# pengpeng-yu/FastPCC

Hardware: AMD Instinct MI355X
Metric: encode+decode Mpoints/sec, lossy_coord_v2 baseline_r1 (stream of 16-frame batches, 2 in flight; one frame at a time = value_one_frame) (higher is better)
Workload: dtype f32; 1 GPU; lossy_coord_v2/baseline_r1 inference, 997645-voxel 1024^3 body-surface frames (cfg#2), seeded random-init weights; one step = a batch of 16 such frames per GPU (15966320 voxels) through compress_many + decompress_many = ONE network traversal over the batch, 16 independent streams; 2 batch(es) in flight per GPU; parallelism=single GPU, 2 batches in flight per GPU on one stream (fastpcc_amd/serving.py), batch_clouds=16, frames_in_flight=2, named_stages=False, bytes=143901, coder_handover_retries=0

## Files before the change

fastpcc_amd/csrc/hip/conv.hip:

```cpp
#include "conv_common.h"
#include <atomic>
#include <cstdlib>

namespace fpcc {
namespace {

template <int NBT, int CH, int WM, int WN>
struct MfmaCfg {
    static constexpr int C_OUT = 32 * NBT;
    static constexpr int TM = 32 * WM;
    static constexpr int NBW = NBT / WN;
    static constexpr int THREADS = 64 * WM * WN;
    static constexpr int G8 = CH / 8;
    static constexpr int W_TOTAL = CH * C_OUT / 4;
    static constexpr int W_PIECES = (W_TOTAL + THREADS - 1) / THREADS;
    static_assert(NBT % WN == 0, "column blocks must divide over the waves");
};

template <typename C, int CH>
__device__ __forceinline__ void fetch_a(const ConvArgs &a, const int32_t *nbr_rows, int cc, int li, int lh,
                                        f32x4 (&ra)[C::G8]) {
    const bool in_x1 = cc * CH < a.c1;
    const float *xb = in_x1 ? a.x1 + cc * CH : a.x2 + (cc * CH - a.c1);
    const int64_t ld = in_x1 ? a.ld1 : a.ld2;
// ... 640 lines not shown
        }
        __builtin_amdgcn_sched_barrier(0);
        for (int s = 0; s < n_stages; ++s) {
            next_stage();
            __builtin_amdgcn_sched_barrier(SB);
#pragma unroll
            for (int g8 = 0; g8 < G8; ++g8) {
                const f32x4 av0 = ra[0][g8], av1 = ra[1][g8];
                const f32x4 b0 = rbv[g8][0], b1 = rbv[g8][1];
#define FPCC_STEP(c)                                                                                     \
                acc[0][0] = __builtin_amdgcn_mfma_f32_32x32x2f32(av0.c, b0.c, acc[0][0], 0, 0, 0);       \
                acc[0][1] = __builtin_amdgcn_mfma_f32_32x32x2f32(av0.c, b1.c, acc[0][1], 0, 0, 0);       \
                acc[1][0] = __builtin_amdgcn_mfma_f32_32x32x2f32(av1.c, b0.c, acc[1][0], 0, 0, 0);       \
                acc[1][1] = __builtin_amdgcn_mfma_f32_32x32x2f32(av1.c, b1.c, acc[1][1], 0, 0, 0);
                FPCC_STEP(x) FPCC_STEP(y) FPCC_STEP(z) FPCC_STEP(w)
#undef FPCC_STEP
                __builtin_amdgcn_sched_barrier(SB);
                ra[0][g8] = *reinterpret_cast<const f32x4 *>(ap[0] + 8 * g8);
                __builtin_amdgcn_sched_barrier(SB);
                ra[1][g8] = *reinterpret_cast<const f32x4 *>(ap[1] + 8 * g8);
#pragma unroll
                for (int nb = 0; nb < 2; ++nb) {
                    __builtin_amdgcn_sched_barrier(SB);
                    rbv[g8][nb] = *reinterpret_cast<const f32x4 *>(bp + ((int64_t)g8 * nbt + nb) * 256);
                }
                __builtin_amdgcn_sched_barrier(SB);
            }
        }
    }

    const float slope = (a.act == FPCC_ACT_PRELU && a.slope) ? a.slope[0] : 0.0f;
    float bias2[2];
#pragma unroll
    for (int nb = 0; nb < 2; ++nb) bias2[nb] = a.bias ? a.bias[32 * ((int)cg * 2 + nb) + li] : 0.0f;
#pragma unroll
    for (int rb = 0; rb < 2; ++rb) {
        int64_t dsts[16];
#pragma unroll
        for (int reg = 0; reg < 16; ++reg) {
            const int64_t o = __shfl(my_row, 32 * rb + (reg & 3) + 8 * (reg >> 2) + 4 * lh);
            dsts[reg] = o < 0 ? -1 : a.out_map ? (int64_t)a.out_map[o * a.om_os + g * a.om_gs] : o * a.groups + g;
        }
#pragma unroll
        for (int reg = 0; reg < 16; ++reg) {
            const int64_t dst = dsts[reg];
            if (dst < 0) continue;
#pragma unroll
            for (int nb = 0; nb < 2; ++nb)
                a.out[dst * a.ldo + 32 * ((int)cg * 2 + nb) + li] = finish(acc[rb][nb][reg], bias2[nb], a.act, slope, a.clip);
        }
    }
}

__global__ __launch_bounds__(256) void k_pack_weights(const float *__restrict__ w, int64_t n_mats, int c_in, int c_out,
                                                      float *__restrict__ wp) {
    const int64_t e = (int64_t)blockIdx.x * 256 + threadIdx.x;
    const int64_t per_mat = (int64_t)c_in * c_out;
    if (e >= n_mats * per_mat) return;
    const int nbt = c_out / 32;
    const int64_t m = e / per_mat;
    int64_t r = e - m * per_mat;
    const int j = (int)(r & 3); r >>= 2;
    const int i = (int)(r & 31); r >>= 5;
    const int h = (int)(r & 1); r >>= 1;
    const int nb = (int)(r % nbt); r /= nbt;
    const int g8 = (int)(r & 3); r >>= 2;
    const int cc = (int)r;
    wp[e] = w[m * per_mat + (int64_t)(32 * cc + 8 * g8 + 4 * h + j) * c_out + 32 * nb + i];
}

inline bool aligned16(const void *p) { return (reinterpret_cast<uintptr_t>(p) & 15) == 0; }

int mfma_chunk(int c1, int c2, int c_out) {
    if (c_out != 32 && c_out != 64 && c_out != 128) return 0;
    const int c_in = c1 + c2;
    if (c_in % 32 == 0 && c1 % 32 == 0) return 32;
    if (c_in % 16 == 0 && c1 % 16 == 0) return 16;
    return 0;
}

int knob(int k);

template <int NBT, int CH, int WM, int WN>
int launch_mfma_cfg(ConvArgs a, hipStream_t s) {
    constexpr int TM = 32 * WM;
    const unsigned tiles = (unsigned)((a.n_out + TM - 1) / TM);
    const dim3 grid(tiles, a.groups), block(64 * WM * WN);
    hipLaunchKernelGGL((k_conv_mfma<NBT, CH, WM, WN>), grid, block, 0, s, a);
    return check_hip(hipGetLastError(), "k_conv_mfma");
}

enum { kKnobWaveOn = 0, kKnobWaveNbw = 1, kKnobWaveSb = 2, kKnobStamps = 3, kKnobGroupedFoldRows = 4, kKnobMfmaCfg = 5, kKnobPointwiseRows = 6,
       kKnobGroupedOff = 7, kKnobGroupedNbw = 8, kKnobWave22Rows = 9, kKnobLdsRows = 10, kKnobLdsRowBlocks = 11, kKnobPersist = 12, kKnobCount = 13 };
int g_knob[kKnobCount] = {-1, -1, -1, -1, -1, -1, -1, -1, -1, -1, -1, -1, -1};
int knob(int k) {
    if (g_knob[k] < 0) {
        static const char *names[kKnobCount] = {"FPCC_CONV_WAVE", "FPCC_WAVE_NBW", "FPCC_WAVE_SB", "", "FPCC_GROUPED_FOLD_ROWS",
                                                "FPCC_MFMA_TILE", "FPCC_POINTWISE_MIN_ROWS", "", "FPCC_GROUPED_NBW",
                                                "FPCC_WAVE22_MIN_ROWS", "FPCC_LDS_MIN_ROWS", "FPCC_LDS_ROW_BLOCKS",
                                                "FPCC_CONV_PERSIST"};
        static const int defaults[kKnobCount] = {1, 0, 1, 0, 100 * 1024, 0, 32 * 1024, 0, 0, 0, 0, 2, 0};
        const char *e = names[k][0] ? getenv(names[k]) : nullptr;
        g_knob[k] = e ? atoi(e) : defaults[k];
    }
    return g_knob[k];
}

template <int NBT, int CH>
int launch_mfma(const ConvArgs &a, hipStream_t s) {
    const int forced = knob(kKnobMfmaCfg) - 1;
    const int64_t work = a.n_out * a.groups;
    constexpr int WNS = NBT >= 2 ? 2 : 1;
    const int cfg = forced >= 0 ? forced : (NBT <= 2 && work >= 128 * 1024) ? 0 : work >= 32 * 1024 ? 1 : 2;
    if (cfg == 0) return launch_mfma_cfg<NBT, CH, 4, 1>(a, s);
    if (cfg == 1) return launch_mfma_cfg<NBT, CH, 2, WNS>(a, s);
    return launch_mfma_cfg<NBT, CH, 1, NBT>(a, s);
}

__global__ __launch_bounds__(256) void k_conv_c1_pointwise(ConvArgs a) {
    const int64_t e = (int64_t)blockIdx.x * 256 + threadIdx.x;
    if (e >= a.n_out * a.c_out) return;
    const int64_t o = e / a.c_out;
    const int j = (int)(e - o * a.c_out);
    const float slope = (a.act == FPCC_ACT_PRELU && a.slope) ? a.slope[0] : 0.0f;
    a.out[o * a.ldo + j] = finish(fmaf(a.x1[o * a.ld1], a.w[j], 0.0f), a.bias ? a.bias[j] : 0.0f, a.act, slope, a.clip);
}

template <int NBW>
int launch_wave_cfg(const ConvArgs &a, const float *wp, int nbt, hipStream_t s) {
    const int64_t row_blocks = (a.n_out + 31) / 32;
    const int64_t units = row_blocks * (nbt / NBW);
    if (units > 0x7fffffffll) return fail_arg("conv_f32: too many work units");
    const dim3 grid((unsigned)((units + 3) / 4), a.groups);
    if (knob(kKnobWaveSb)) hipLaunchKernelGGL((k_conv_wave<NBW, 32, 0x6>), grid, dim3(256), 0, s, a, wp, nbt, (unsigned)units);
    else hipLaunchKernelGGL((k_conv_wave<NBW, 32, 0>), grid, dim3(256), 0, s, a, wp, nbt, (unsigned)units);
    return check_hip(hipGetLastError(), "k_conv_wave");
}

constexpr int kMaxDevices = 16;
inline int current_device() {
    int dev = 0;
    return (hipGetDevice(&dev) == hipSuccess && dev >= 0 && dev < kMaxDevices) ? dev : -1;
}
int cu_count() {
    static std::atomic<int> cached[kMaxDevices];
    const int dev = current_device();
    if (dev < 0) return 256;
    int n = cached[dev].load(std::memory_order_relaxed);
    if (n == 0) {
        hipDeviceProp_t prop;
        n = (hipGetDeviceProperties(&prop, dev) == hipSuccess && prop.multiProcessorCount > 0) ? prop.multiProcessorCount : 256;
        cached[dev].store(n, std::memory_order_relaxed);
    }
    return n;
// ... 21 lines not shown
    *rc = check_hip(hipMemsetD32Async(reinterpret_cast<hipDeviceptr_t>(c), (int)start, 1, s), "unit counter fill");
    return c;
}

inline int64_t persist_slots() {
    const int v = knob(kKnobPersist);
    return v > 16 ? v : (int64_t)v * cu_count();
}
inline bool persist_ok(const ConvArgs &a) {
    return knob(kKnobPersist) > 0 && a.nbr && a.nbr_ks == 1 && (a.nbr_os & 3) == 0 && a.nbr_os >= ((a.n_off + 3) & ~3) &&
           (reinterpret_cast<uintptr_t>(a.nbr) & 15) == 0 && a.groups == 1;
}

template <int NBW>
int launch_grouped_cfg(const ConvArgs &a, const float *wp, int nbt, hipStream_t s) {
    const int64_t row_blocks = (a.n_out + 31) / 32;
    const int64_t units = row_blocks * (nbt / NBW);
    if (units > 0x7fffffffll) return fail_arg("conv_f32: too many work units");
    const bool stamps = knob(kKnobStamps) != 0;
    const int64_t slots = persist_slots();
    if (!stamps && persist_ok(a) && units > slots) {
        int rc = FPCC_OK;
        unsigned *counter = next_unit_counter((unsigned)slots, s, &rc);
        if (rc != FPCC_OK) return rc;
        hipLaunchKernelGGL((k_conv_wave<NBW, 32, 0x6, false, 4, false, true>), dim3((unsigned)slots, 1), dim3(256), 0, s, a, wp, nbt, (unsigned)units,
                           counter);
        return check_hip(hipGetLastError(), "k_conv_wave(grouped, persistent)");
    }
    if (stamps)
        hipLaunchKernelGGL((k_conv_wave<NBW, 32, 0x6, true, 4>), dim3((unsigned)units, a.groups), dim3(256), 0, s, a, wp, nbt, (unsigned)units);
    else
        hipLaunchKernelGGL((k_conv_wave<NBW, 32, 0x6, false, 4>), dim3((unsigned)units, a.groups), dim3(256), 0, s, a, wp, nbt, (unsigned)units);
    return check_hip(hipGetLastError(), "k_conv_wave(grouped)");
}

template <int NBW>
int launch_folded_cfg(const ConvArgs &a, const float *wp, int nbt, hipStream_t s) {
    const int64_t units = ((a.n_out + 31) / 32) * (nbt / NBW);
    if (units > 0x7fffffffll) return fail_arg("conv_f32: too many work units");
    const int64_t slots = persist_slots();
    if (!knob(kKnobStamps) && persist_ok(a) && (units + 3) / 4 > slots) {
        int rc = FPCC_OK;
        unsigned *counter = next_unit_counter((unsigned)(4 * slots), s, &rc);
        if (rc != FPCC_OK) return rc;
        hipLaunchKernelGGL((k_conv_wave<NBW, 32, 0x6, false, 1, true, true>), dim3((unsigned)slots, 1), dim3(256), 0, s, a, wp, nbt, (unsigned)units,
                           counter);
        return check_hip(hipGetLastError(), "k_conv_wave(folded, persistent)");
    }
    hipLaunchKernelGGL((k_conv_wave<NBW, 32, 0x6, false, 1, true>), dim3((unsigned)((units + 3) / 4), a.groups), dim3(256), 0, s, a, wp, nbt,
                       (unsigned)units);
    return check_hip(hipGetLastError(), "k_conv_wave(folded)");
}

int launch_grouped(const ConvArgs &a, const float *wp, hipStream_t s) {
    const int nbt = a.c_out / 32;
    const int64_t lds_rows = knob(kKnobLdsRows);
    if (lds_rows > 0 && a.n_out >= lds_rows) {
        const int rc = launch_conv_lds(a, wp, knob(kKnobLdsRowBlocks), knob(kKnobStamps) != 0, s);
        if (rc != -1) return rc;
    }
    const int64_t fold_rows = knob(kKnobGroupedFoldRows);
    if (fold_rows > 0 && a.n_out >= fold_rows && knob(kKnobGroupedNbw) <= 0)
        return nbt % 2 == 0 ? launch_folded_cfg<2>(a, wp, nbt, s) : launch_folded_cfg<1>(a, wp, nbt, s);
    int nbw = knob(kKnobGroupedNbw);
    if (nbw <= 0) nbw = a.n_out >= 40 * 1024 ? 2 : 1;
    while (nbw > nbt || nbt % nbw) nbw >>= 1;
    return nbw == 2 ? launch_grouped_cfg<2>(a, wp, nbt, s) : launch_grouped_cfg<1>(a, wp, nbt, s);
}

int launch_wave22(const ConvArgs &a, const float *wp, int nbt, hipStream_t s) {
    const int64_t units = ((a.n_out + 63) / 64) * (nbt / 2);
    if (units > 0x7fffffffll) return fail_arg("conv_f32: too many work units");
    const dim3 grid((unsigned)((units + 3) / 4), a.groups);
    if (knob(kKnobWaveSb)) hipLaunchKernelGGL((k_conv_wave22<0x6>), grid, dim3(256), 0, s, a, wp, nbt, (unsigned)units);
    else hipLaunchKernelGGL((k_conv_wave22<0>), grid, dim3(256), 0, s, a, wp, nbt, (unsigned)units);
    return check_hip(hipGetLastError(), "k_conv_wave22");
}

int launch_wave(const ConvArgs &a, const float *wp, hipStream_t s) {
    const int nbt = a.c_out / 32;
    const int64_t work = a.n_out * a.groups;
    const int64_t rows22 = knob(kKnobWave22Rows);
    if (rows22 > 0 && a.n_off > 1 && nbt % 2 == 0 && work >= rows22 && knob(kKnobWaveNbw) <= 0) return launch_wave22(a, wp, nbt, s);
    int nbw = knob(kKnobWaveNbw);
    if (nbw <= 0) nbw = work >= 32 * 1024 ? 2 : 1;
    while (nbw > nbt || nbt % nbw) nbw >>= 1;
    if (nbw >= 4) return launch_wave_cfg<4>(a, wp, nbt, s);
    if (nbw == 2) return launch_wave_cfg<2>(a, wp, nbt, s);
    return launch_wave_cfg<1>(a, wp, nbt, s);
}


template <int NBW, int NCH>
__global__ __launch_bounds__(256, 2) void k_pointwise_wave(ConvArgs a, const float *__restrict__ wp, int nbt, unsigned n_row_blocks,
                                                           unsigned waves_per_cg) {
    constexpr int AC = NCH < 4 ? NCH : 4;
    constexpr int TW = 32 * NBW + 4;
    __shared__ float s_tile[4][32 * TW];
    const int lane = threadIdx.x & 63, wv = threadIdx.x >> 6;
    const int li = lane & 31, lh = lane >> 5;
    const unsigned n_cg = (unsigned)(nbt / NBW);
    const unsigned w = blockIdx.x * 4u + (unsigned)wv;
    const unsigned cg = w % n_cg, slot = w / n_cg;
    if (slot >= waves_per_cg) return;

    f32x4 rb[NCH][4][NBW];
    {
        const float *wpl = wp + ((int64_t)cg * NBW) * 256 + lane * 4;
#pragma unroll
        for (int cc = 0; cc < NCH; ++cc)
#pragma unroll
            for (int g8 = 0; g8 < 4; ++g8)
#pragma unroll
                for (int nb = 0; nb < NBW; ++nb)
                    rb[cc][g8][nb] = *reinterpret_cast<const f32x4 *>(wpl + (((int64_t)cc * 4 + g8) * nbt + nb) * 256);
    }
// ... 183 lines not shown
    return check_hip(hipGetLastError(), "k_conv_valu");
}

}
}

using namespace fpcc;

static bool use_grouped(int c1, int c2, int c_out, int n_offsets, int groups) {
    return mfma_chunk(c1, c2, c_out) == 32 && n_offsets >= 8 && n_offsets <= kMaxOffsets && groups == 1 && !knob(kKnobGroupedOff);
}

extern "C" int fpcc_conv_f32_order(int c1, int c2, int c_out) { return mfma_chunk(c1, c2, c_out) ? 1 : 0; }

extern "C" int64_t fpcc_conv_f32_ws_bytes(int c1, int c2, int c_out, int n_offsets, int groups, int64_t n_out) {
    if (n_out > 0 && use_grouped(c1, c2, c_out, n_offsets, groups)) return (int64_t)n_offsets * (c1 + c2) * c_out * 4;
    return 0;
}

extern "C" int fpcc_conv_f32_order_ex(int c1, int c2, int c_out, int n_offsets, int groups, int64_t n_out) {
    (void)n_out;
    if (use_grouped(c1, c2, c_out, n_offsets, groups)) return 3;
    return mfma_chunk(c1, c2, c_out) ? 1 : 0;
}

extern "C" int fpcc_numerics_version(void) { return FPCC_NUMERICS_VERSION; }

extern "C" int fpcc_conv_ones_k3_f32(const uint32_t *masks, int64_t n, const float *w, const float *bias, int c_out, int act,
                                     const float *slope, float clip, float *out, int ldo, void *stream) {
    if (n < 0 || c_out < 4 || c_out > 32 || c_out % 4 || ldo < c_out || ldo % 4) return fail_arg("conv_ones_k3: 4 <= c_out <= 32, multiple of 4");
    if (n == 0) return FPCC_OK;
    if (!masks || !w || !out || !aligned16(out)) return fail_arg("conv_ones_k3: null or unaligned pointer");
    if (act == FPCC_ACT_PRELU && !slope) return fail_arg("conv_ones_k3: PReLU needs a slope pointer");
    hipStream_t st = as_stream(stream);
    switch (c_out) {
        case 4: return launch_ones_k3<4>(masks, n, w, bias, act, slope, clip, out, ldo, st);
        case 8: return launch_ones_k3<8>(masks, n, w, bias, act, slope, clip, out, ldo, st);
        case 12: return launch_ones_k3<12>(masks, n, w, bias, act, slope, clip, out, ldo, st);
        case 16: return launch_ones_k3<16>(masks, n, w, bias, act, slope, clip, out, ldo, st);
        case 20: return launch_ones_k3<20>(masks, n, w, bias, act, slope, clip, out, ldo, st);
        case 24: return launch_ones_k3<24>(masks, n, w, bias, act, slope, clip, out, ldo, st);
        case 28: return launch_ones_k3<28>(masks, n, w, bias, act, slope, clip, out, ldo, st);
        default: return launch_ones_k3<32>(masks, n, w, bias, act, slope, clip, out, ldo, st);
    }
}

extern "C" int fpcc_conv_debug_stamps(unsigned long long *buf, int64_t n_u64) {
    if (n_u64 < 0 || (n_u64 > 0 && !buf)) return fail_arg("conv_debug_stamps: null buffer");
    const long long cap = buf ? n_u64 : 0;
    FPCC_HIP(hipMemcpyToSymbol(HIP_SYMBOL(g_stamp_buf), &buf, sizeof(buf)));
    FPCC_HIP(hipMemcpyToSymbol(HIP_SYMBOL(g_stamp_cap), &cap, sizeof(cap)));
    return set_lds_stamp_buffer(buf, cap);
}

extern "C" int fpcc_conv_set_tuning(int which, int value) {
    if (which < 0 || which >= kKnobCount) return fail_arg("conv_set_tuning: unknown knob");
    if (which == kKnobGroupedOff) {
        const char *e = getenv("FPCC_EXPERIMENT");
        if (!e || atoi(e) != 1)
            return fail_arg("conv_set_tuning: the summation order is part of the stream format (FPCC_EXPERIMENT=1 to override)");
    }
    if (which == kKnobStamps && value != 0 && value != 16)
        return fail_arg("conv_set_tuning: knob 3 is 0 or 16 (stamped builds); the timing ablations are no longer part of the library");
    const int before = knob(which);
    g_knob[which] = value < 0 ? 0 : value;
    return before;
}

extern "C" int64_t fpcc_conv_packed_floats(int c1, int c2, int c_out, int n_offsets, int groups) {
    if (mfma_chunk(c1, c2, c_out) != 32 || n_offsets < 1 || n_offsets > kMaxOffsets || groups < 1) return 0;
    return (int64_t)groups * n_offsets * (c1 + c2) * c_out;
}

extern "C" int fpcc_conv_pack_weights_f32(const float *w, int64_t n_mats, int c_in, int c_out, float *w_packed, void *stream) {
    if (n_mats < 0 || c_in < 32 || c_in % 32 || (c_out != 32 && c_out != 64 && c_out != 128))
        return fail_arg("conv_pack_weights: c_in must be a multiple of 32 and c_out one of 32, 64, 128");
    if (n_mats == 0) return FPCC_OK;
    if (!w || !w_packed) return fail_arg("conv_pack_weights: null pointer");
    hipLaunchKernelGGL(k_pack_weights, dim3(blocks_for(n_mats * c_in * c_out, 256)), dim3(256), 0, as_stream(stream), w, n_mats,
                       c_in, c_out, w_packed);
    return check_hip(hipGetLastError(), "k_pack_weights");
}

extern "C" int fpcc_conv_f32(const float *x1, int c1, int ld1, const float *x2, int c2, int ld2, const int32_t *nbr,
                             int n_offsets, int64_t nbr_ks, int64_t nbr_os, const float *w, const float *bias, int c_out,
                             int groups, const int32_t *out_map, int64_t om_os, int64_t om_gs, float *out, int ldo,
                             int64_t n_out, int act, const float *slope, float clip, const int32_t *row_order,
                             void *ws, int64_t ws_bytes, void *stream) {
    return fpcc_conv_f32_pk(x1, c1, ld1, x2, c2, ld2, nbr, n_offsets, nbr_ks, nbr_os, w, nullptr, bias, c_out, groups, out_map,
                            om_os, om_gs, out, ldo, n_out, act, slope, clip, row_order, ws, ws_bytes, stream);
}

namespace fpcc {
PendingEvents &pending_events() {
    static thread_local PendingEvents p;
    return p;
}
}

extern "C" int fpcc_time_next_launch(void *start_event, void *end_event) {
    PendingEvents &p = pending_events();
    p.ev0 = start_event;
    p.ev1 = end_event;
    return FPCC_OK;
}

// ... 383 lines not shown
```

fastpcc_amd/hipops.py:

```python
import collections
import ctypes as C
import functools
from typing import List, Optional, Sequence, Tuple

import torch

from . import _native

_vp, _i64, _i32, _f32 = C.c_void_p, C.c_int64, C.c_int, C.c_float

ACT_NONE, ACT_PRELU, ACT_RELU = 0, 1, 2

_SIGS = {
    'fpcc_morton3d_encode': (_i32, [_vp, _i64, _i64, _i32, _i32, _i32, _vp, _vp]),
    'fpcc_hilbert3d_encode': (_i32, [_vp, _i64, _i64, _i32, _i32, _i32, _i32, _vp, _vp]),
    'fpcc_keys_from_coords': (_i32, [_vp, _i64, _i32, _i32, _vp, _vp]),
    'fpcc_coords_from_keys': (_i32, [_vp, _i64, _i32, _i32, _vp, _vp, _vp]),
    'fpcc_sort_keys': (_i64, [_vp, _i64, _i32, _vp, _vp, _vp, _i64, _vp]),
    'fpcc_unique_keys': (_i64, [_vp, _i64, _vp, _vp, _vp, _vp, _i64, _vp]),
    'fpcc_coarsen': (_i64, [_vp, _i64, _vp, _vp, _vp, _vp, _vp, _i64, _vp]),
    'fpcc_octree_level': (_i64, [_vp, _i64, _i64, _i32, _vp, _vp, _vp, _vp, _i64, _vp, _vp, _i64, _vp]),
    'fpcc_level_histogram': (_i64, [_vp, _i64, _i32, _vp, _vp]),
    'fpcc_level_histogram_clouds': (_i64, [_vp, _i64, _i32, _i32, _i32, _vp, _vp]),
    'fpcc_refine': (_i64, [_vp, _i64, _vp, _vp, _vp, _vp, _vp, _vp, _i64, _vp]),
    'fpcc_nbr27_search': (_i32, [_vp, _i64, _i32, _vp, _vp]),
    'fpcc_nbr27_from_parent': (_i32, [_vp, _vp, _i64, _vp, _i64, _vp, _vp, _vp]),
    'fpcc_nbr27_from_parent_ex': (_i32, [_vp, _vp, _i64, _vp, _i64, _vp, _vp, _vp, _vp, _vp]),
    'fpcc_conv_row_keys_masks': (_i32, [_vp, _i64, _i32, _vp, _vp]),
    'fpcc_gather_table_rows_i32': (_i32, [_vp, _i32, _vp, _i64, _vp, _vp]),
    'fpcc_mask27_from_parent': (_i32, [_vp, _vp, _i64, _vp, _i64, _vp, _vp, _vp]),
    'fpcc_conv_ones_k3_f32': (_i32, [_vp, _i64, _vp, _vp, _i32, _i32, _vp, C.c_float, _vp, _i32, _vp]),
    'fpcc_conv_f32': (_i32, [_vp, _i32, _i32, _vp, _i32, _i32, _vp, _i32, _i64, _i64, _vp, _vp, _i32, _i32,
                             _vp, _i64, _i64, _vp, _i32, _i64, _i32, _vp, _f32, _vp, _vp, _i64, _vp]),
    'fpcc_conv_f32_pk': (_i32, [_vp, _i32, _i32, _vp, _i32, _i32, _vp, _i32, _i64, _i64, _vp, _vp, _vp, _i32, _i32,
                                _vp, _i64, _i64, _vp, _i32, _i64, _i32, _vp, _f32, _vp, _vp, _i64, _vp]),
    'fpcc_conv_set_tuning': (_i32, [_i32, _i32]),
    'fpcc_conv_debug_stamps': (_i32, [_vp, _i64]),
    'fpcc_conv_i8_debug_stamps': (_i32, [_vp, _i64]),
    'fpcc_time_next_launch': (_i32, [_vp, _vp]),
    'fpcc_transpose_table_i32': (_i32, [_vp, _i32, _i64, _vp, _i32, _vp]),
    'fpcc_numerics_version': (_i32, []),
    'fpcc_conv_packed_floats': (_i64, [_i32, _i32, _i32, _i32, _i32]),
    'fpcc_conv_pack_weights_f32': (_i32, [_vp, _i64, _i32, _i32, _vp, _vp]),
    'fpcc_nn_dist2': (_i32, [_vp, _i64, _i32, _vp, _i64, _vp, _vp, _vp]),
    'fpcc_knn3d': (_i32, [_vp, _i64, _vp, _i64, _i32, _vp, _vp, _vp]),
    'fpcc_sum_i64': (_i32, [_vp, _i64, _vp, _vp]),
    'fpcc_knn_voxels': (_i32, [_vp, _i64, _i32, _vp, _i64, _i32, _i32, _vp, _vp, _vp]),
    'fpcc_pca_normals': (_i32, [_vp, _i64, _i32, _vp, _i64, _i32, _vp, _vp]),
    'fpcc_nn_plane_dist2': (_i32, [_vp, _i64, _i32, _vp, _vp, _i64, _vp, _vp, _vp, _vp]),
    'fpcc_transfer_normals_ws_bytes': (_i64, [_i64, _i64]),
    'fpcc_transfer_normals': (_i32, [_vp, _i64, _vp, _vp, _vp, _i64, _vp, _i32, _vp, _vp, _i64, _vp]),
    'fpcc_sum_max_f64': (_i32, [_vp, _i64, _vp, _vp, _i64, _vp]),
    'fpcc_recolor_ws_bytes': (_i64, [_i64]),
    'fpcc_recolor': (_i32, [_vp, _i64, _vp, _i64, _vp, _i32, _vp, _vp, _i64, _vp]),
    'fpcc_keys_member': (_i32, [_vp, _i64, _vp, _i64, _vp, _vp]),
    'fpcc_transpose_weights_f32': (_i32, [_vp, _i32, _i32, _i32, _i32, _vp, _vp]),
    'fpcc_conv_wgrad_ws_bytes': (_i64, [_i32, _i32, _i32, _i32, _i64]),
    'fpcc_conv_wgrad_f32': (_i32, [_vp, _i32, _i32, _vp, _i32, _i32, _vp, _i32, _i64, _i64, _vp, _i64, _i64, _i32, _i64, _vp, _vp,
                                   _i32, _vp, _i64, _vp]),
    'fpcc_epilogue_bwd_ws_bytes': (_i64, [_i64, _i32]),
    'fpcc_epilogue_bwd_f32': (_i32, [_vp, _i32, _vp, _i32, _i64, _i32, _i32, _vp, _vp, _i32, _vp, _vp, _vp, _i64, _vp]),
    'fpcc_noisy_normal_ws_bytes': (_i64, [_i64]),
    'fpcc_noisy_normal_bits_f32': (_i32, [_vp, _vp, _i64, _f32, _f32, _f32, _vp, _vp, _vp, _vp, _i64, _vp]),
    'fpcc_deep_factorized_ws_bytes': (_i64, [_i64, _i32]),
    'fpcc_deep_factorized_bits_f32': (_i32, [_vp, _i64, _i32, _i32, _vp, _vp, _vp, _f32, _vp, _i32, _vp, _vp, _i64, _vp]),
    'fpcc_conv_tile_keys': (_i32, [_vp, _i32, _vp, _i64, _i32, _vp, _vp]),
    'fpcc_conv_regroup_rows': (_i32, [_vp, _vp, _i64, _i32, _vp, _vp]),
    'fpcc_conv_group_order': (_i32, [_vp, _i64, _vp, _vp]),
    'fpcc_conv_row_keys': (_i32, [_vp, _i32, _i64, _i64, _i64, _i32, _vp, _vp, _vp]),
    'fpcc_conv_f32_ws_bytes': (_i64, [_i32, _i32, _i32, _i32, _i32, _i64]),
    'fpcc_conv_f32_order': (_i32, [_i32, _i32, _i32]),
    'fpcc_conv_f32_order_ex': (_i32, [_i32, _i32, _i32, _i32, _i32, _i64]),
    'fpcc_gather_sum_f32': (_i32, [_vp, _i32, _vp, _i32, _i64, _i64, _i64, _vp, _i32, _vp, _f32, _vp, _vp]),
    'fpcc_gather_sum_generated_f32': (_i32, [_vp, _i32, _vp, _i64, _vp, _i32, _vp, _f32, _vp, _vp]),
    'fpcc_logit_to_prob16': (_i32, [_vp, _i64, _vp, _vp]),
    'fpcc_quantize_symbols': (_i32, [_vp, _i64, _f32, _vp, _vp]),
    'fpcc_child_mask': (_i32, [_vp, _i64, _vp, _vp]),
    'fpcc_topk_keep': (_i64, [_vp, _i64, _i64, _vp, _vp, _i64, _vp]),
    'fpcc_topk_keep_cells': (_i64, [_vp, _i64, _vp, _i64, _i64, _vp, _vp, _i64, _vp]),
    'fpcc_topk_keep_batch': (_i64, [_vp, _i64, _vp, _i32, _vp, _i64, _vp, _vp, _vp, _i64, _vp]),
    'fpcc_gather_rows_f32': (_i32, [_vp, _i32, _i32, _vp, _i64, _vp, _i32, _vp]),
    'fpcc_compact_coords': (_i64, [_vp, _i64, _vp, _i32, _i32, _vp, _vp, _vp, _vp, _i64, _vp]),
    'fpcc_int_init': (_i32, []),
    'fpcc_hash_insert_coords': (_i32, [_vp, _vp, _i64, _vp, _i64, _vp]),
    'fpcc_hash_lookup_coords': (_i32, [_vp, _vp, _i64, _vp, _i64, _vp, _vp, _vp, _vp]),
    'fpcc_hash_insert_coords_bxyz': (_i32, [_vp, _vp, _i64, _vp, _i64, _vp]),
    'fpcc_hash_lookup_coords_bxyz': (_i32, [_vp, _vp, _i64, _vp, _i64, _vp, _vp, _vp, _vp]),
    'fpcc_hash_insert_keys': (_i32, [_vp, _vp, _i64, _vp, _i64, _vp]),
    'fpcc_hash_lookup_keys': (_i32, [_vp, _vp, _i64, _vp, _i64, _vp, _vp]),
# ... 318 lines not shown
    _ok(lib().fpcc_mask27_from_parent(_dev(keys, torch.int64, 'keys', True), _dev(parent_of, torch.int32, 'parent_of', True),
                                      n, _dev(parent_nbr, torch.int32, 'parent_nbr'), m,
                                      _dev(child_row, torch.int32, 'child_row', True), masks.data_ptr(), _stream()))
    return masks


def conv_ones_k3(masks: torch.Tensor, w: torch.Tensor, c_out: int, *, bias: Optional[torch.Tensor] = None, act: int = 0,
                 slope: Optional[torch.Tensor] = None, clip: float = 0.0) -> torch.Tensor:
    n = masks.shape[0]
    if w.numel() != 27 * c_out or not w.is_contiguous():
        raise ValueError('weights must be contiguous [27, 1, c_out]')
    out = torch.empty((n, c_out), dtype=torch.float32, device=masks.device)
    _ok(lib().fpcc_conv_ones_k3_f32(_dev(masks, torch.int32, 'masks'), n, _dev(w, torch.float32, 'w'),
                                    _dev(bias, torch.float32, 'bias', True), c_out, act, _dev(slope, torch.float32, 'slope', True),
                                    float(clip), out.data_ptr(), c_out, _stream()))
    return out



def _rows2d(t: torch.Tensor, name: str):
    if t.dim() != 2 or t.dtype != torch.float32 or not t.is_cuda or t.stride(1) != 1:
        raise TypeError(f'{name} must be a 2-D float32 GPU tensor with unit column stride')
    return t.data_ptr(), t.shape[1], (t.stride(0) if t.shape[0] > 1 else max(t.shape[1], t.stride(0)))


_PACKED: 'collections.OrderedDict' = collections.OrderedDict()
_PACKED_MAX = 1024


def packed_weights(w: torch.Tensor, c1: int, c2: int, c_out: int, n_offsets: int, groups: int, fresh: bool = False) -> Optional[torch.Tensor]:
    if not lib().fpcc_conv_packed_floats(c1, c2, c_out, n_offsets, groups):
        return None
    if fresh:
        out = torch.empty(w.numel(), dtype=torch.float32, device=w.device)
        _ok(lib().fpcc_conv_pack_weights_f32(w.data_ptr(), groups * n_offsets, c1 + c2, c_out, out.data_ptr(), _stream()))
        return out
    key = (w.data_ptr(), w.numel(), c1 + c2, c_out)
    ent = _PACKED.get(key)
    if ent is not None and ent[1] == w._version:
        _PACKED.move_to_end(key)
        return ent[2]
    out = torch.empty(w.numel(), dtype=torch.float32, device=w.device)
    _ok(lib().fpcc_conv_pack_weights_f32(w.data_ptr(), groups * n_offsets, c1 + c2, c_out, out.data_ptr(), _stream()))
    _PACKED[key] = (w, w._version, out)
    while len(_PACKED) > _PACKED_MAX:
        _PACKED.popitem(last=False)
    return out


KNOB_WAVE_ON, KNOB_WAVE_NBW, KNOB_WAVE_SB, KNOB_WAVE_DBG, KNOB_MFMA_TILE, KNOB_POINTWISE_ROWS = 0, 1, 2, 3, 5, 6
KNOB_GROUPED_FOLD_ROWS = 4
KNOB_GROUPED_OFF, KNOB_GROUPED_NBW, KNOB_WAVE22_ROWS = 7, 8, 9
KNOB_PERSIST = 12
KNOB_LDS_ROWS, KNOB_LDS_ROW_BLOCKS = 10, 11


def numerics_version() -> int:
    return lib().fpcc_numerics_version()


def clock_probe(out2: torch.Tensor, spin_us: int = 20) -> None:
    _ok(lib().fpcc_clock_probe(_dev(out2, torch.int64, 'out2'), int(spin_us), _stream()))


def transpose_table(table: torch.Tensor, ld: int = 32) -> torch.Tensor:
    k, n = table.shape
    out = torch.empty((n, ld), dtype=torch.int32, device=table.device)
    _ok(lib().fpcc_transpose_table_i32(_dev(table, torch.int32, 'table', n == 0), k, n, out.data_ptr(), ld, _stream()))
    return out


def conv_debug_stamps(buf: Optional[torch.Tensor]) -> None:
    if buf is None:
        _ok(lib().fpcc_conv_debug_stamps(None, 0))
    else:
        _ok(lib().fpcc_conv_debug_stamps(_dev(buf, torch.int64, 'buf'), buf.numel()))


def conv_i8_debug_stamps(buf: Optional[torch.Tensor]) -> None:
    if buf is None:
        _ok(lib().fpcc_conv_i8_debug_stamps(None, 0))
    else:
        _ok(lib().fpcc_conv_i8_debug_stamps(_dev(buf, torch.int64, 'buf'), buf.numel()))


def conv_set_tuning(which: int, value: int) -> int:
    before = _ok(lib().fpcc_conv_set_tuning(int(which), int(value)))
    conv_order.cache_clear()
    return before


CONV_TRACE = None
TRACE_LOCK = __import__('threading').RLock()
CLOCK_HOOK = None
_EVENT_POOL: list = []
_trace_tls = __import__('threading').local()


def set_thread_trace(trace) -> None:
    global _n_thread_traces
    had = getattr(_trace_tls, 'trace', None) is not None
    _trace_tls.trace = trace
    with TRACE_LOCK:
        _n_thread_traces += (trace is not None) - had


_n_thread_traces = 0
# ... 887 lines not shown
```

include/fpcc_hip.h:

```cpp
#ifndef FPCC_HIP_H_
#define FPCC_HIP_H_
#include <stdint.h>
#ifdef __cplusplus
extern "C" {
#endif

typedef enum {
    FPCC_OK = 0,
    FPCC_E_ARG = -1,
    FPCC_E_HIP = -2,
    FPCC_E_WORKSPACE = -3
} fpcc_status;

const char *fpcc_last_error(void);
int fpcc_device_count(void);
int fpcc_clock_probe(int64_t *out2, int spin_us, void *stream);


int fpcc_morton3d_encode(const int32_t *coords, int64_t n, int64_t row_stride, int col_bit0, int col_bit1, int col_bit2,
                         int64_t *keys_out, void *stream);

int fpcc_hilbert3d_encode(const int32_t *coords, int64_t n, int64_t row_stride, int col_x, int col_y, int col_z, int bits,
                          int64_t *keys_out, void *stream);

int fpcc_keys_from_coords(const int32_t *coords, int64_t n, int level, int bits, int64_t *keys_out, void *stream);
int fpcc_coords_from_keys(const int64_t *keys, int64_t n, int level, int bits, const int32_t *offset_xyz,
                          int32_t *coords_out, void *stream);

int64_t fpcc_sort_keys(const int64_t *keys_in, int64_t n, int end_bit, int64_t *keys_out, int32_t *perm_out,
                       void *ws, int64_t ws_bytes, void *stream);

int64_t fpcc_unique_keys(const int64_t *keys, int64_t n, int64_t *ukeys_out, int32_t *first_out, int32_t *count_out,
                         void *ws, int64_t ws_bytes, void *stream);

int64_t fpcc_coarsen(const int64_t *keys, int64_t n, int32_t *parent_of, int64_t *pkeys, int32_t *child_row,
                     int32_t *count_out, void *ws, int64_t ws_bytes, void *stream);
int64_t fpcc_octree_level(const int64_t *keys, int64_t n, int64_t m, int batch_shift, int64_t *pkeys, int32_t *coords, int32_t *bits,
                          int32_t *table, int64_t table_rows, int16_t *symbols, void *ws, int64_t ws_bytes, void *stream);
int64_t fpcc_level_histogram(const int64_t *keys, int64_t n, int levels, int32_t *hist, void *stream);
int64_t fpcc_level_histogram_clouds(const int64_t *keys, int64_t n, int levels, int cloud_shift, int n_clouds, int32_t *hist,
                                    void *stream);

int64_t fpcc_refine(const int64_t *pkeys, int64_t m, const uint8_t *mask, int64_t *keys_out, int32_t *parent_of,
                    int32_t *child_row, int32_t *count_out, void *ws, int64_t ws_bytes, void *stream);

int fpcc_nbr27_search(const int64_t *keys, int64_t n, int bits, int32_t *nbr, void *stream);
int fpcc_nbr27_from_parent(const int64_t *keys, const int32_t *parent_of, int64_t n, const int32_t *parent_nbr,
                           int64_t m, const int32_t *child_row, int32_t *nbr, void *stream);
int fpcc_nbr27_from_parent_ex(const int64_t *keys, const int32_t *parent_of, int64_t n, const int32_t *parent_nbr, int64_t m,
                              const int32_t *child_row, int32_t *nbr, int32_t *rows_out, uint32_t *masks_out, void *stream);
int fpcc_mask27_from_parent(const int64_t *keys, const int32_t *parent_of, int64_t n, const int32_t *parent_nbr, int64_t m,
                            const int32_t *child_row, uint32_t *masks_out, void *stream);

enum { FPCC_ACT_NONE = 0, FPCC_ACT_PRELU = 1, FPCC_ACT_RELU = 2 };

#define FPCC_NUMERICS_VERSION 3
#define FPCC_PAD_MIN_ROWS 8192
int fpcc_numerics_version(void);

int fpcc_conv_f32(const float *x1, int c1, int ld1, const float *x2, int c2, int ld2,
                  const int32_t *nbr, int n_offsets, int64_t nbr_ks, int64_t nbr_os,
                  const float *w, const float *bias, int c_out, int groups,
                  const int32_t *out_map, int64_t om_os, int64_t om_gs, float *out, int ldo, int64_t n_out,
                  int act, const float *slope, float clip, const int32_t *row_order, void *ws, int64_t ws_bytes,
                  void *stream);
int64_t fpcc_conv_packed_floats(int c1, int c2, int c_out, int n_offsets, int groups);
int fpcc_conv_set_tuning(int which, int value);
int fpcc_conv_debug_stamps(unsigned long long *buf, int64_t n_u64);
int fpcc_time_next_launch(void *start_event, void *end_event);
int fpcc_conv_i8_debug_stamps(unsigned long long *buf, int64_t n_u64);

int fpcc_conv_ones_k3_f32(const uint32_t *masks, int64_t n, const float *w, const float *bias, int c_out, int act,
                          const float *slope, float clip, float *out, int ldo, void *stream);
int fpcc_conv_pack_weights_f32(const float *w, int64_t n_mats, int c_in, int c_out, float *w_packed, void *stream);
int fpcc_conv_f32_pk(const float *x1, int c1, int ld1, const float *x2, int c2, int ld2,
                     const int32_t *nbr, int n_offsets, int64_t nbr_ks, int64_t nbr_os,
                     const float *w, const float *w_packed, const float *bias, int c_out, int groups,
                     const int32_t *out_map, int64_t om_os, int64_t om_gs, float *out, int ldo, int64_t n_out,
                     int act, const float *slope, float clip, const int32_t *row_order, void *ws, int64_t ws_bytes,
                     void *stream);
#define FPCC_MLP_CHAIN_MAX_LAYERS 4
typedef struct {
    const float *w;
    const float *w_packed;
    const float *bias;
    const float *slope;
    int c_out;
    int act;
    float clip;
} fpcc_mlp_layer;
typedef struct {
    const float *x; int cx; int ldx;
    const float *y; int cy; int ldy;
    int cat_layer;
    int n_layers;
    fpcc_mlp_layer layers[FPCC_MLP_CHAIN_MAX_LAYERS];
    float *out; int ldo;
    int64_t n;
} fpcc_mlp_chain;
int fpcc_mlp_chain_f32(const fpcc_mlp_chain *chain, void *stream);
int fpcc_mlp_chain_set_form(int form);
int fpcc_pointwise_head_f32(const float *x, int c0, int ldx, const float *w1, const float *b1, int c1, int act1,
                            const float *slope1, int order1, const float *w2, const float *b2, int act2, const float *slope2,
                            float clip, float *out, int64_t n, void *stream);
int fpcc_conv_row_keys(const int32_t *nbr, int n_offsets, int64_t nbr_ks, int64_t nbr_os, int64_t n, int window_log2,
                       int64_t *keys_out, uint32_t *masks_out, void *stream);
int fpcc_conv_row_keys_masks(const uint32_t *masks, int64_t n, int window_log2, int64_t *keys_out, void *stream);
int fpcc_gather_table_rows_i32(const int32_t *rows, int ld, const int32_t *order, int64_t n, int32_t *out, void *stream);
int fpcc_conv_tile_keys(const uint32_t *row_masks, int n_offsets, const int32_t *row_order, int64_t n, int group,
                        int64_t *keys_out, void *stream);
int fpcc_conv_group_order(const int64_t *group_keys, int64_t n_groups, int32_t *perm_out, void *stream);
int fpcc_conv_regroup_rows(const int32_t *row_order, const int32_t *group_perm, int64_t n, int group, int32_t *row_order_out,
                           void *stream);
int64_t fpcc_conv_f32_ws_bytes(int c1, int c2, int c_out, int n_offsets, int groups, int64_t n_out);
int fpcc_conv_f32_order(int c1, int c2, int c_out);
int fpcc_conv_f32_order_ex(int c1, int c2, int c_out, int n_offsets, int groups, int64_t n_out);

int64_t fpcc_conv_wgrad_ws_bytes(int c_in, int c_out, int n_offsets, int groups, int64_t n);
int fpcc_conv_wgrad_f32(const float *x, int c_in, int ldx, const float *dy, int c_out, int ldy,
                        const int32_t *nbr, int n_offsets, int64_t nbr_ks, int64_t nbr_os,
// ... 156 lines not shown
```

Baseline: 89.59 Mpoints/s.

## Add 64-row folded grouped conv kernel for large row-ordered layers

Adds a new folded grouped-convolution MFMA kernel in which each wave handles 64 output rows and two 32-column blocks (a 2x2 block of 32x32 accumulators). Each loaded weight fragment is reused across two row blocks and each activation fragment across two column blocks. The kernel is selected by default for large grouped layers (row_order set, at least 200K rows, full offset count, 64 or 128 output channels). In exchange it holds more accumulators per wave (launch bounds 256 with 2 blocks), which may lower occupancy. A launch counter is also added for verification.

```diff
diff --git a/fastpcc_amd/csrc/hip/conv.hip b/fastpcc_amd/csrc/hip/conv.hip
--- a/fastpcc_amd/csrc/hip/conv.hip
+++ b/fastpcc_amd/csrc/hip/conv.hip
@@ -716,6 +716,209 @@
     }
 }
 
+__global__ __launch_bounds__(256, 2) void k_conv_fold64(ConvArgs a, const float *__restrict__ wp, int nbt, unsigned n_units) {
+    constexpr int CH = 32, G8 = 4;
+    constexpr int SB = 0x6;
+    __shared__ int32_t s_nbr_all[4][kMaxOffsets * 64];
+
+    const int lane = threadIdx.x & 63, wv = __builtin_amdgcn_readfirstlane(threadIdx.x >> 6);
+    const int li = lane & 31, lh = lane >> 5;
+    const unsigned n_cg = (unsigned)(nbt / 2);
+    const unsigned blk = a.row_order ? blockIdx.x : xcd_remap(blockIdx.x, gridDim.x);
+    const unsigned unit = blk * 4u + (unsigned)wv;
+    if (unit >= n_units) return;
+    const unsigned rb_ = unit / n_cg, cg = unit - rb_ * n_cg;
+    const int64_t row0 = (int64_t)rb_ * 64;
+    const int c_in = a.c1 + a.c2;
+    const int n_chunks = c_in / CH;
+    const int n_off = a.n_off;
+    int32_t *s_nbr = s_nbr_all[wv];
+
+    int32_t my_row = -1;
+    if (row0 + lane < a.n_out) my_row = a.row_order ? a.row_order[row0 + lane] : (int32_t)(row0 + lane);
+    unsigned wmask = 0;
+    if (table_is_row_major(a)) {
+        const int64_t p = row0 + lane < a.n_out ? row0 + lane : a.n_out - 1;
+        const i32x4 *rowp = reinterpret_cast<const i32x4 *>(a.nbr + p * a.nbr_os);
+        const int last_piece = (n_off - 1) >> 2;
+        i32x4 q[7];
+#pragma unroll
+        for (int j = 0; j < 7; ++j) q[j] = rowp[min(j, last_piece)];
+#pragma unroll
+        for (int j = 0; j < 7; ++j)
+#pragma unroll
+            for (int e = 0; e < 4; ++e) {
+                const int k = 4 * j + e;
+                if (k >= kMaxOffsets) continue;
+                const int32_t v = (k < n_off && my_row >= 0) ? q[j][e] : -1;
+                if (k < n_off) s_nbr[k * 64 + lane] = v;
+                if (__ballot(v >= 0) != 0ull) wmask |= 1u << k;
+            }
+    } else {
+        for (int k = 0; k < n_off; ++k) {
+            int32_t v = -1;
+            if (my_row >= 0) v = a.nbr[(int64_t)k * a.nbr_ks + (int64_t)my_row * a.nbr_os];
+            s_nbr[k * 64 + lane] = v;
+            if (__ballot(v >= 0) != 0ull) wmask |= 1u << k;
+        }
+    }
+    __builtin_amdgcn_wave_barrier();
+    wmask = __builtin_amdgcn_readfirstlane(wmask);
+
+    f32x16 acc[2][2], tsum[2][2];
+#pragma unroll
+    for (int rb = 0; rb < 2; ++rb)
+#pragma unroll
+        for (int nb = 0; nb < 2; ++nb)
+#pragma unroll
+            for (int r = 0; r < 16; ++r) acc[rb][nb][r] = 0.0f;
+
+    int n_folded = 0, cur_g = 0;
+    auto fold_acc = [&]() {
+#pragma unroll
+        for (int rb = 0; rb < 2; ++rb)
+#pragma unroll
+            for (int nb = 0; nb < 2; ++nb)
+#pragma unroll
+                for (int r = 0; r < 16; ++r) {
+                    tsum[rb][nb][r] = n_folded ? tsum[rb][nb][r] + acc[rb][nb][r] : acc[rb][nb][r];
+                    acc[rb][nb][r] = 0.0f;
+                }
+        ++n_folded;
+    };
+    auto fold_zero = [&]() {
+#pragma unroll
+        for (int rb = 0; rb < 2; ++rb)
+#pragma unroll
+            for (int nb = 0; nb < 2; ++nb)
+#pragma unroll
+                for (int r = 0; r < 16; ++r) tsum[rb][nb][r] = n_folded ? tsum[rb][nb][r] + 0.0f : 0.0f;
+        ++n_folded;
+    };
+    unsigned rest_c = wmask;
+    int cc_c = 0;
+    if (wmask) {
+        cur_g = offset_group_of(__ffs(wmask) - 1, n_off);
+        for (int gz = 0; gz < cur_g; ++gz) fold_zero();
+    }
+
+    const int n_stages = __popc(wmask) * n_chunks;
+    if (n_stages > 0) {
+        const int64_t chunk_floats = (int64_t)G8 * nbt * 256;
+        const float *wp_g = wp + ((int64_t)cg * 2) * 256 + lane * 4;
+        const float *const zero = (const float *)g_zero_row + 4 * lh;
+        const float *const x1b = a.x1 + 4 * lh, *const x2b = a.x2 ? a.x2 + 4 * lh : zero;
+        const int64_t ld1 = a.ld1, ld2 = a.ld2;
+        const int n1 = a.c1 / CH;
+        const float *a1[2], *a2[2], *bpk;
+        int step[2];
+        auto set_offset = [&](int k) {
+#pragma unroll
+            for (int rb = 0; rb < 2; ++rb) {
+                const int32_t idx = s_nbr[k * 64 + 32 * rb + li];
+                const int32_t neg = idx >> 31;
+                const uint64_t m = (uint64_t)(int64_t)neg, z = reinterpret_cast<uint64_t>(zero) & m;
+                const int64_t row = idx & ~neg;
+                a1[rb] = reinterpret_cast<const float *>((reinterpret_cast<uint64_t>(x1b + row * ld1) & ~m) | z);
+                a2[rb] = reinterpret_cast<const float *>((reinterpret_cast<uint64_t>(x2b + row * ld2) & ~m) | z);
+                step[rb] = CH & ~neg;
+            }
+            bpk = wp_g + (int64_t)k * n_chunks * chunk_floats;
+        };
+        unsigned rest = wmask;
+        int cc_f = 0;
+        set_offset(__ffs(rest) - 1);
+        const float *ap[2], *bp;
+        auto next_stage = [&]() {
+            const bool in1 = cc_f < n1;
+            const int c = in1 ? cc_f : cc_f - n1;
+            ap[0] = (in1 ? a1[0] : a2[0]) + c * step[0];
+            ap[1] = (in1 ? a1[1] : a2[1]) + c * step[1];
+            bp = bpk + cc_f * chunk_floats;
+            if (cc_f + 1 < n_chunks) {
+                ++cc_f;
+            } else {
+                const unsigned r2 = rest & (rest - 1);
+                if (r2) { rest = r2; cc_f = 0; set_offset(__ffs(r2) - 1); }
+            }
+        };
+        f32x4 ra[2][G8], rbv[G8][2];
+        next_stage();
+#pragma unroll
+        for (int g8 = 0; g8 < G8; ++g8) {
+            __builtin_amdgcn_sched_barrier(0);
+            ra[0][g8] = *reinterpret_cast<const f32x4 *>(ap[0] + 8 * g8);
+            __builtin_amdgcn_sched_barrier(0);
+            ra[1][g8] = *reinterpret_cast<const f32x4 *>(ap[1] + 8 * g8);
+#pragma unroll
+            for (int nb = 0; nb < 2; ++nb) {
+                __builtin_amdgcn_sched_barrier(0);
+                rbv[g8][nb] = *reinterpret_cast<const f32x4 *>(bp + ((int64_t)g8 * nbt + nb) * 256);
+            }
+        }
+        __builtin_amdgcn_sched_barrier(0);
+        for (int s = 0; s < n_stages; ++s) {
+            if (cc_c == 0) {
+                const int gk = offset_group_of(__ffs(rest_c) - 1, n_off);
+                if (gk != cur_g) {
+                    fold_acc();
+                    for (int gz = cur_g + 1; gz < gk; ++gz) fold_zero();
+                    cur_g = gk;
+                }
+            }
+            if (++cc_c == n_chunks) { cc_c = 0; rest_c &= rest_c - 1; }
+            next_stage();
+            __builtin_amdgcn_sched_barrier(SB);
+#pragma unroll
+            for (int g8 = 0; g8 < G8; ++g8) {
+                const f32x4 av0 = ra[0][g8], av1 = ra[1][g8];
+                const f32x4 b0 = rbv[g8][0], b1 = rbv[g8][1];
+#define FPCC_STEP(c)                                                                                     \
+                acc[0][0] = __builtin_amdgcn_mfma_f32_32x32x2f32(av0.c, b0.c, acc[0][0], 0, 0, 0);       \
+                acc[0][1] = __builtin_amdgcn_mfma_f32_32x32x2f32(av0.c, b1.c, acc[0][1], 0, 0, 0);       \
+                acc[1][0] = __builtin_amdgcn_mfma_f32_32x32x2f32(av1.c, b0.c, acc[1][0], 0, 0, 0);       \
+                acc[1][1] = __builtin_amdgcn_mfma_f32_32x32x2f32(av1.c, b1.c, acc[1][1], 0, 0, 0);
+                FPCC_STEP(x) FPCC_STEP(y) FPCC_STEP(z) FPCC_STEP(w)
+#undef FPCC_STEP
+                __builtin_amdgcn_sched_barrier(SB);
+                ra[0][g8] = *reinterpret_cast<const f32x4 *>(ap[0] + 8 * g8);
+                __builtin_amdgcn_sched_barrier(SB);
+                ra[1][g8] = *reinterpret_cast<const f32x4 *>(ap[1] + 8 * g8);
+#pragma unroll
+                for (int nb = 0; nb < 2; ++nb) {
+                    __builtin_amdgcn_sched_barrier(SB);
+                    rbv[g8][nb] = *reinterpret_cast<const f32x4 *>(bp + ((int64_t)g8 * nbt + nb) * 256);
+                }
+                __builtin_amdgcn_sched_barrier(SB);
+            }
+        }
+    }
+    if (wmask) { fold_acc(); ++cur_g; }
+    for (int gz = cur_g; gz < 4; ++gz) fold_zero();
+
+    const float slope = (a.act == FPCC_ACT_PRELU && a.slope) ? a.slope[0] : 0.0f;
+    float bias2[2];
+#pragma unroll
+    for (int nb = 0; nb < 2; ++nb) bias2[nb] = a.bias ? a.bias[32 * ((int)cg * 2 + nb) + li] : 0.0f;
+#pragma unroll
+    for (int rb = 0; rb < 2; ++rb) {
+        int64_t dsts[16];
+#pragma unroll
+        for (int reg = 0; reg < 16; ++reg) {
+            const int64_t o = __shfl(my_row, 32 * rb + (reg & 3) + 8 * (reg >> 2) + 4 * lh);
+            dsts[reg] = o < 0 ? -1 : o;
+        }
+#pragma unroll
+        for (int reg = 0; reg < 16; ++reg) {
+            const int64_t dst = dsts[reg];
+            if (dst < 0) continue;
+#pragma unroll
+            for (int nb = 0; nb < 2; ++nb)
+                a.out[dst * a.ldo + 32 * ((int)cg * 2 + nb) + li] = finish(tsum[rb][nb][reg], bias2[nb], a.act, slope, a.clip);
+        }
+    }
+}
+
 __global__ __launch_bounds__(256) void k_pack_weights(const float *__restrict__ w, int64_t n_mats, int c_in, int c_out,
                                                       float *__restrict__ wp) {
     const int64_t e = (int64_t)blockIdx.x * 256 + threadIdx.x;
@@ -755,15 +958,15 @@
 }
 
 enum { kKnobWaveOn = 0, kKnobWaveNbw = 1, kKnobWaveSb = 2, kKnobStamps = 3, kKnobGroupedFoldRows = 4, kKnobMfmaCfg = 5, kKnobPointwiseRows = 6,
-       kKnobGroupedOff = 7, kKnobGroupedNbw = 8, kKnobWave22Rows = 9, kKnobLdsRows = 10, kKnobLdsRowBlocks = 11, kKnobPersist = 12, kKnobCount = 13 };
-int g_knob[kKnobCount] = {-1, -1, -1, -1, -1, -1, -1, -1, -1, -1, -1, -1, -1};
+       kKnobGroupedOff = 7, kKnobGroupedNbw = 8, kKnobWave22Rows = 9, kKnobLdsRows = 10, kKnobLdsRowBlocks = 11, kKnobPersist = 12, kKnobFold64 = 13, kKnobCount = 14 };
+int g_knob[kKnobCount] = {-1, -1, -1, -1, -1, -1, -1, -1, -1, -1, -1, -1, -1, -1};
 int knob(int k) {
     if (g_knob[k] < 0) {
         static const char *names[kKnobCount] = {"FPCC_CONV_WAVE", "FPCC_WAVE_NBW", "FPCC_WAVE_SB", "", "FPCC_GROUPED_FOLD_ROWS",
                                                 "FPCC_MFMA_TILE", "FPCC_POINTWISE_MIN_ROWS", "", "FPCC_GROUPED_NBW",
                                                 "FPCC_WAVE22_MIN_ROWS", "FPCC_LDS_MIN_ROWS", "FPCC_LDS_ROW_BLOCKS",
-                                                "FPCC_CONV_PERSIST"};
-        static const int defaults[kKnobCount] = {1, 0, 1, 0, 100 * 1024, 0, 32 * 1024, 0, 0, 0, 0, 2, 0};
+                                                "FPCC_CONV_PERSIST", "FPCC_CONV_FOLD64"};
+        static const int defaults[kKnobCount] = {1, 0, 1, 0, 100 * 1024, 0, 32 * 1024, 0, 0, 0, 0, 2, 0, 0};
         const char *e = names[k][0] ? getenv(names[k]) : nullptr;
         g_knob[k] = e ? atoi(e) : defaults[k];
     }
@@ -891,6 +1094,23 @@
     return check_hip(hipGetLastError(), "k_conv_wave(folded)");
 }
 
+constexpr int64_t kFold64Rows = 200 * 1024;
+std::atomic<long long> g_fold64_launches{0};
+inline bool use_fold64(const ConvArgs &a, int nbt) {
+    if ((nbt != 2 && nbt != 4) || a.n_off != kMaxOffsets || knob(kKnobPersist) > 0) return false;
+    const int v = knob(kKnobFold64);
+    if (v) return v >= 2;
+    return a.row_order && a.n_out >= kFold64Rows;
+}
+
+int launch_fold64(const ConvArgs &a, const float *wp, int nbt, hipStream_t s) {
+    const int64_t units = ((a.n_out + 63) / 64) * (nbt / 2);
+    if (units > 0x7fffffffll) return fail_arg("conv_f32: too many work units");
+    hipLaunchKernelGGL(k_conv_fold64, dim3((unsigned)((units + 3) / 4), 1), dim3(256), 0, s, a, wp, nbt, (unsigned)units);
+    g_fold64_launches.fetch_add(1, std::memory_order_relaxed);
+    return check_hip(hipGetLastError(), "k_conv_fold64");
+}
+
 int launch_grouped(const ConvArgs &a, const float *wp, hipStream_t s) {
     const int nbt = a.c_out / 32;
     const int64_t lds_rows = knob(kKnobLdsRows);
@@ -899,8 +1119,10 @@
         if (rc != -1) return rc;
     }
     const int64_t fold_rows = knob(kKnobGroupedFoldRows);
-    if (fold_rows > 0 && a.n_out >= fold_rows && knob(kKnobGroupedNbw) <= 0)
+    if (fold_rows > 0 && a.n_out >= fold_rows && knob(kKnobGroupedNbw) <= 0) {
+        if (use_fold64(a, nbt)) return launch_fold64(a, wp, nbt, s);
         return nbt % 2 == 0 ? launch_folded_cfg<2>(a, wp, nbt, s) : launch_folded_cfg<1>(a, wp, nbt, s);
+    }
     int nbw = knob(kKnobGroupedNbw);
     if (nbw <= 0) nbw = a.n_out >= 40 * 1024 ? 2 : 1;
     while (nbw > nbt || nbt % nbw) nbw >>= 1;
@@ -1190,6 +1412,8 @@
     FPCC_HIP(hipMemcpyToSymbol(HIP_SYMBOL(g_stamp_cap), &cap, sizeof(cap)));
     return set_lds_stamp_buffer(buf, cap);
 }
+
+extern "C" long long fpcc_conv_fold64_launches(void) { return g_fold64_launches.load(std::memory_order_relaxed); }
 
 extern "C" int fpcc_conv_set_tuning(int which, int value) {
     if (which < 0 || which >= kKnobCount) return fail_arg("conv_set_tuning: unknown knob");
diff --git a/fastpcc_amd/hipops.py b/fastpcc_amd/hipops.py
--- a/fastpcc_amd/hipops.py
+++ b/fastpcc_amd/hipops.py
@@ -35,6 +35,7 @@
     'fpcc_conv_f32_pk': (_i32, [_vp, _i32, _i32, _vp, _i32, _i32, _vp, _i32, _i64, _i64, _vp, _vp, _vp, _i32, _i32,
                                 _vp, _i64, _i64, _vp, _i32, _i64, _i32, _vp, _f32, _vp, _vp, _i64, _vp]),
     'fpcc_conv_set_tuning': (_i32, [_i32, _i32]),
+    'fpcc_conv_fold64_launches': (_i64, []),
     'fpcc_conv_debug_stamps': (_i32, [_vp, _i64]),
     'fpcc_conv_i8_debug_stamps': (_i32, [_vp, _i64]),
     'fpcc_time_next_launch': (_i32, [_vp, _vp]),
@@ -459,7 +460,12 @@
 KNOB_GROUPED_FOLD_ROWS = 4
 KNOB_GROUPED_OFF, KNOB_GROUPED_NBW, KNOB_WAVE22_ROWS = 7, 8, 9
 KNOB_PERSIST = 12
+KNOB_FOLD64 = 13
 KNOB_LDS_ROWS, KNOB_LDS_ROW_BLOCKS = 10, 11
+
+
+def conv_fold64_launches() -> int:
+    return int(lib().fpcc_conv_fold64_launches())
 
 
 def numerics_version() -> int:
diff --git a/include/fpcc_hip.h b/include/fpcc_hip.h
--- a/include/fpcc_hip.h
+++ b/include/fpcc_hip.h
@@ -66,6 +66,7 @@
                   void *stream);
 int64_t fpcc_conv_packed_floats(int c1, int c2, int c_out, int n_offsets, int groups);
 int fpcc_conv_set_tuning(int which, int value);
+long long fpcc_conv_fold64_launches(void);
 int fpcc_conv_debug_stamps(unsigned long long *buf, int64_t n_u64);
 int fpcc_time_next_launch(void *start_event, void *end_event);
 int fpcc_conv_i8_debug_stamps(unsigned long long *buf, int64_t n_u64);
```

Result: faster. 92.03 Mpoints/s (median of 6 runs) (+2.7%).
